# pfe-rs/lk-s-2022-estimacija-pokreta

Measured on AMD Instinct MI355X. Metric: Mpix/s flow (1024x436, bcd_times=4), higher is better.
Workload: dtype f64; 1 GPU; single 1024x436 Sintel-shape pair per step per GPU, forward only, bcd_times=4 (BASELINE.json configs[1]); cells 64x27, 150 labels/px; pairs_in_flight_per_gpu=7, mode=batch

## Files before the change

lk-s-2022-estimacija-pokreta_amd/csrc/bcd.hip:

```cpp
#include "dflow_common.h"

#define BCD_THREADS 192
#ifndef BCD_MINWAVES
#define BCD_MINWAVES 5
#endif
#define BCD_MASK_WORDS 5
#define BCD_BLK 5
#define BCD_LIST 15
#define BCD_LDS_LABELS 256
#define BCD_TB_STEPS 32
#define BCD_GROUPS 3
#define BCD_CAP_B01 40
#define BCD_CAP_B2 16
#define BCD_CAP_C01 24
#define BCD_CAP_C2 8
#define BCD_ROW_B (2 * BCD_CAP_B01 + BCD_CAP_B2)
#define BCD_ROW_C (2 * BCD_CAP_C01 + BCD_CAP_C2)
#define BCD_ROW_BC (BCD_ROW_B + BCD_ROW_C + 2)
#define BCD_POOL_DIV 32

#define BLK_MORE 0x800u
#define BLK_HAS_B 0x8000u
#define BLK_HAS_C 0x80000u
#define BLK_EMPTY_X 0xFFFFFFFFu
#define BLK_EMPTY_Y 0x000000FFu

__device__ static inline void chain_geom(int phase, int chain, int H, int W, int &ty, int &tx, int &ys, int &xs, int &len)
{
    if (phase == 0) { ty = 0; tx = 2 * chain; ys = 1; xs = 0; len = H; }
    else if (phase == 1) { ty = 2 * chain; tx = W - 1; ys = 0; xs = -1; len = W; }
    else if (phase == 2) { ty = H - 1; tx = (W / 2) * 2 - 1 - 2 * chain; ys = -1; xs = 0; len = H; }
    else { ty = (H / 2) * 2 - 1 - 2 * chain; tx = 0; ys = 0; xs = 1; len = W; }
}

struct BcdPlanes {
    uint8_t *back;
    uint2 *lab;
    uint2 *blkA;
    uint2 *blkBC;
    uint32_t *masks;
    uint32_t *cursor;
    uint32_t pool_rows;
};

__global__ void __launch_bounds__(256) bcd_lists_kernel(int H, int W, int LP, int tpsi, const uint32_t *__restrict__ proposals,
                                                        const float *__restrict__ lcosts, const int32_t *__restrict__ nprop,
                                                        BcdPlanes pl)
{
    __shared__ uint32_t s_cols[4][256];
    __shared__ __attribute__((aligned(16))) uint8_t s_list[4][64][16];
    const int lane = threadIdx.x & 63, wv = threadIdx.x >> 6;
    const int q = (int)blockIdx.x * 4 + __builtin_amdgcn_readfirstlane(wv);
    if (q >= H * W) return;
    const int y = q / W, x = q % W;
    const int py = (x & 1) ? y + 1 : y - 1, sy = (x & 1) ? y - 1 : y + 1;
    const int px = (y & 1) ? x - 1 : x + 1, sx = (y & 1) ? x + 1 : x - 1;
    const bool start0 = py < 0 || py >= H, start1 = px < 0 || px >= W;
    const bool v0 = sy >= 0 && sy < H, v1 = sx >= 0 && sx < W;
    const int p0 = v0 ? sy * W + x : q, p1 = v1 ? y * W + sx : q;
    const int pn = nprop[q], tn0 = v0 ? nprop[p0] : 0, tn1 = v1 ? nprop[p1] : 0;
    const int half = lane >> 5;
    uint32_t fq[3], f[5];
#pragma unroll
    for (int j = 0; j < 3; j++) {
        const int k = lane + 64 * j;
        fq[j] = k < pn ? flow_bias(proposals[(size_t)q * LP + k]) : 0u;
        s_cols[wv][k] = fq[j];
    }
    s_cols[wv][192 + lane] = 0u;
#pragma unroll
    for (int j = 0; j < 2; j++) {
        const int k = lane + 64 * j;
        f[j] = k < tn0 ? flow_bias(proposals[(size_t)p0 * LP + k]) : 0u;
        f[2 + j] = k < tn1 ? flow_bias(proposals[(size_t)p1 * LP + k]) : 0u;
    }
    {
        const int k = 128 + (lane & 31);
        f[4] = k < (half ? tn1 : tn0) ? flow_bias(proposals[(size_t)(half ? p1 : p0) * LP + k]) : 0u;
    }
#pragma unroll
    for (int j = 0; j < 3; j++) {
        const int k = lane + 64 * j;
        if (k < LP) pl.lab[(size_t)q * LP + k] = make_uint2(fq[j], __float_as_uint(k < pn ? lcosts[(size_t)q * LP + k] : DFLOW_FILL_COST));
    }
    if (start0 || start1) {
#pragma unroll
        for (int j = 0; j < 3; j++) {
            const int k = lane + 64 * j;
            if (k < LP) {
                if (start0) pl.blkA[((size_t)q * 2 + 0) * LP + k] = make_uint2(BLK_EMPTY_X, BLK_EMPTY_Y);
                if (start1) pl.blkA[((size_t)q * 2 + 1) * LP + k] = make_uint2(BLK_EMPTY_X, BLK_EMPTY_Y);
            }
        }
    }
    if (!v0 && !v1) return;
    const uint32_t kbias = 0x80000000u - (uint32_t)tpsi;
    const uint32_t *__restrict__ colp = proposals + (size_t)q * LP;
    uint32_t m[5][BCD_MASK_WORDS];
    const bool fifth = LP > 128 && (tn0 > 128 || tn1 > 128);
    auto build = [&](auto with5) {
#pragma unroll
        for (int j = 0; j < BCD_MASK_WORDS; j++) {
#pragma unroll
            for (int g = 0; g < 5; g++) m[g][j] = 0xFFFFFFFFu;
            if (32 * j < pn) {
                const int nv = pn - 32 * j;
                auto cols8 = [&](auto hic) {
#pragma unroll
                    for (int cc = decltype(hic)::value; cc > decltype(hic)::value - 8; cc--) {
                        const uint32_t col = flow_bias(colp[32 * j + cc]);
#pragma unroll
                        for (int g = 0; g < 4; g++) m[g][j] = __builtin_amdgcn_alignbit(m[g][j], __builtin_amdgcn_sad_u16(col, f[g], kbias), 31);
                        if (decltype(with5)::value) m[4][j] = __builtin_amdgcn_alignbit(m[4][j], __builtin_amdgcn_sad_u16(col, f[4], kbias), 31);
                    }
                };
                if (nv > 24) cols8(IntC<31>());
                if (nv > 16) cols8(IntC<23>());
                if (nv > 8) cols8(IntC<15>());
                cols8(IntC<7>());
                if (nv < 32 && (nv & 7) != 0) {
                    const uint32_t inval = ~0u << nv;
#pragma unroll
                    for (int g = 0; g < 5; g++) m[g][j] |= inval;
                }
            }
        }
    };
    if (fifth) build(IntC<1>()); else build(IntC<0>());

    auto emit = [&](auto mergedc, const uint32_t (&mg)[BCD_MASK_WORDS], const uint32_t me, const int ig, const int tl, const int tn,
                    const bool valid, const size_t pd) {
        constexpr bool MERGED = decltype(mergedc)::value != 0;
        uint32_t w[BCD_MASK_WORDS];
        int cnt = 0;
        uint32_t dead = valid && tl < tn ? 0u : ~0u;
        asm("" : "+v"(dead));
#pragma unroll
        for (int j = 0; j < BCD_MASK_WORDS; j++) { w[j] = __builtin_amdgcn_bitop3_b32(mg[j], dead, 0u, 0x03); cnt += __popc(w[j]); }
        uint8_t *row = &s_list[wv][lane][0];
        *reinterpret_cast<uint4 *>(row) = make_uint4(0xFFFFFFFFu, 0xFFFFFFFFu, 0xFFFFFFFFu, 0xFFFFFFFFu);
        const int n = min(cnt, BCD_LIST);
        const bool any = __ballot(cnt > 0) != 0ull;
        if (any) {
            uint32_t wt[BCD_MASK_WORDS];
#pragma unroll
            for (int j = 0; j < BCD_MASK_WORDS; j++) wt[j] = w[j];
            if (__ballot(cnt > BCD_LIST)) {
                int extra = cnt - BCD_LIST;
#pragma unroll
                for (int j = BCD_MASK_WORDS - 1; j >= 0; j--)
                    while (extra > 0 && wt[j]) { wt[j] &= ~(0x80000000u >> __clz(wt[j])); extra--; }
            }
            uint8_t *ap = row;
#pragma unroll
            for (int j = 0; j < BCD_MASK_WORDS; j++) {
                uint32_t ww = wt[j];
                while (ww) { *ap++ = (uint8_t)(32 * j + __ffs(ww) - 1); ww &= ww - 1; }
            }
        }
        const uint4 lst = *reinterpret_cast<const uint4 *>(row);
        const uint32_t l0 = lst.x, l1 = lst.y, l2 = lst.z, l3 = lst.w;
        uint32_t c0 = 0u, c1 = 0u;
        if (any) {
            auto slots = [&](auto lo, auto hi) {
#pragma unroll
                for (int e = decltype(lo)::value; e < decltype(hi)::value; e++) {
                    const uint32_t word = e < 4 ? l0 : (e < 8 ? l1 : (e < 12 ? l2 : l3));
                    const uint32_t k = (word >> (8 * (e & 3))) & 0xFFu;
                    const uint32_t psi = flow_l1_biased(me, s_cols[wv][k]);
                    if (e < 8) c0 |= psi << (4 * e); else c1 |= psi << (4 * (e - 8));
                }
            };
            slots(IntC<0>(), IntC<BCD_BLK>());
            if (__ballot(n > BCD_BLK)) {
                slots(IntC<BCD_BLK>(), IntC<2 * BCD_BLK>());
                if (__ballot(n > 2 * BCD_BLK)) slots(IntC<2 * BCD_BLK>(), IntC<BCD_LIST>());
            }
        }
        const unsigned long long pp = (((unsigned long long)c1 << 32) | c0) & ~(~0ull << (4 * n));
        const unsigned long long hasB = __ballot(cnt > BCD_BLK), hasC = __ballot(cnt > 2 * BCD_BLK);
        uint32_t rankB = __builtin_amdgcn_mbcnt_hi((uint32_t)(hasB >> 32), __builtin_amdgcn_mbcnt_lo((uint32_t)hasB, 0u));
        uint32_t rankC = __builtin_amdgcn_mbcnt_hi((uint32_t)(hasC >> 32), __builtin_amdgcn_mbcnt_lo((uint32_t)hasC, 0u));
        if (MERGED && half) { rankB -= (uint32_t)__popc((uint32_t)hasB); rankC -= (uint32_t)__popc((uint32_t)hasC); }
        const uint32_t capB = ig < 2 ? BCD_CAP_B01 : BCD_CAP_B2, capC = ig < 2 ? BCD_CAP_C01 : BCD_CAP_C2;
        const bool storeB = cnt > BCD_BLK && rankB < capB, storeC = cnt > 2 * BCD_BLK && storeB && rankC < capC;
        const bool more = cnt > BCD_LIST || (cnt > BCD_BLK && !storeB) || (cnt > 2 * BCD_BLK && !storeC);
        const uint32_t ax = l0;
        const uint32_t ay = (l1 & 0xFFu) | (((uint32_t)pp & 0xFFFFFu) << 8) | (more ? BLK_MORE : 0u) | (storeB ? BLK_HAS_B : 0u) |
                            (storeC ? BLK_HAS_C : 0u) | ((uint32_t)(more ? 15 : min(cnt, 15)) << 28);
        const uint32_t bx = __builtin_amdgcn_alignbit(l2, l1, 8);
        const uint32_t by = ((l2 >> 8) & 0xFFu) | (((uint32_t)(pp >> 20) & 0xFFFFFu) << 8);
        const uint32_t cx = __builtin_amdgcn_alignbit(l3, l2, 16);
        const uint32_t cy = ((l3 >> 16) & 0xFFu) | (((uint32_t)(pp >> 40) & 0xFFFFFu) << 8);
        if (valid && tl < LP) pl.blkA[pd * (size_t)LP + tl] = make_uint2(ax, ay);
        if (storeB) pl.blkBC[pd * BCD_ROW_BC + ig * BCD_CAP_B01 + rankB] = make_uint2(bx, by);
        if (storeC) pl.blkBC[pd * BCD_ROW_BC + BCD_ROW_B + ig * BCD_CAP_C01 + rankC] = make_uint2(cx, cy);
        const unsigned long long dense = __ballot(more);
        if (dense) {
            uint32_t base = 0u;
            if (lane == 0) base = atomicAdd(pl.cursor, (uint32_t)__popcll(dense));
            base = (uint32_t)__builtin_amdgcn_readfirstlane((int)base);
            uint32_t rank = __builtin_amdgcn_mbcnt_hi((uint32_t)(dense >> 32), __builtin_amdgcn_mbcnt_lo((uint32_t)dense, 0u));
            if (MERGED) {
                const uint32_t nlo = (uint32_t)__popc((uint32_t)dense);
                if ((lane & 31) == 0 && (half ? (dense >> 32) != 0ull : (uint32_t)dense != 0u))
                    reinterpret_cast<uint32_t *>(pl.blkBC + pd * BCD_ROW_BC + BCD_ROW_B + BCD_ROW_C)[ig] = base + (half ? nlo : 0u);
            } else if (lane == 0) {
                reinterpret_cast<uint32_t *>(pl.blkBC + pd * BCD_ROW_BC + BCD_ROW_B + BCD_ROW_C)[ig] = base;
            }
            const uint32_t slot = base + rank;
            if (more && slot < pl.pool_rows) {
                uint32_t *out = pl.masks + (size_t)slot * BCD_MASK_WORDS;
#pragma unroll
                for (int j = 0; j < BCD_MASK_WORDS; j++) out[j] = w[j];
            }
        }
    };
    const size_t pd0 = (size_t)p0 * 2 + 0, pd1 = (size_t)p1 * 2 + 1;
    if (v0) {
        emit(IntC<0>(), m[0], f[0], 0, lane, tn0, true, pd0);
        if (LP > 64) emit(IntC<0>(), m[1], f[1], 1, 64 + lane, tn0, true, pd0);
    }
    if (v1) {
        emit(IntC<0>(), m[2], f[2], 0, lane, tn1, true, pd1);
        if (LP > 64) emit(IntC<0>(), m[3], f[3], 1, 64 + lane, tn1, true, pd1);
    }
    if (LP > 128) emit(IntC<1>(), m[4], f[4], 2, 128 + (lane & 31), half ? tn1 : tn0, half ? v1 : v0, half ? pd1 : pd0);
}

#ifndef BCD_MAX_BATCH
#define BCD_MAX_BATCH 8
#endif
struct BcdPass {
    const int32_t *nprop;
    int32_t *bestlabels;
    BcdPlanes pl;
};
struct BcdArgs {
    int H, W, LP, tpsi, phase;
    double lamda;
    BcdPass pass[BCD_MAX_BATCH];
};

struct Cand {
    double v; int k;
};

__device__ static inline void cand_min(Cand &a, double ov, int ok)
{
    const bool take = ov < a.v || (ov == a.v && ok < a.k);
    a.v = take ? ov : a.v;
    a.k = take ? ok : a.k;
}

template <int CTRL> __device__ static inline void cand_dpp(const Cand &a, double &ov, int &ok)
{
    const int lo = __double2loint(a.v), hi = __double2hiint(a.v);
    const int olo = __builtin_amdgcn_update_dpp(lo, lo, CTRL, 0xF, 0xF, false);
    const int ohi = __builtin_amdgcn_update_dpp(hi, hi, CTRL, 0xF, 0xF, false);
    ok = __builtin_amdgcn_update_dpp(a.k, a.k, CTRL, 0xF, 0xF, false);
    ov = __hiloint2double(ohi, olo);
}

#define DPP_ROW_SHL1 0x101
#define DPP_ROW_SHL2 0x102
#define DPP_ROW_SHL4 0x104
#define DPP_ROW_SHL8 0x108

__device__ static inline void wave_min_lane0(Cand &pm)
{
    double ov; int ok;
    cand_dpp<DPP_ROW_SHL1>(pm, ov, ok); cand_min(pm, ov, ok);
    cand_dpp<DPP_ROW_SHL2>(pm, ov, ok); cand_min(pm, ov, ok);
    cand_dpp<DPP_ROW_SHL4>(pm, ov, ok); cand_min(pm, ov, ok);
    cand_dpp<DPP_ROW_SHL8>(pm, ov, ok); cand_min(pm, ov, ok);
    const int lo = __double2loint(pm.v), hi = __double2hiint(pm.v);
#pragma unroll
    for (int r = 1; r < 4; r++) {
        const double rv = __hiloint2double(__builtin_amdgcn_readlane(hi, 16 * r), __builtin_amdgcn_readlane(lo, 16 * r));
        const int rk = __builtin_amdgcn_readlane(pm.k, 16 * r);
        cand_min(pm, rv, rk);
    }
}

__device__ static inline uint32_t wave_u32_min_asm(uint32_t x)
{
    asm volatile("s_nop 1\n\t"
                 "v_min_u32_dpp %0, %0, %0 row_shl:1 row_mask:0xf bank_mask:0xf\n\t"
                 "s_nop 1\n\t"
                 "v_min_u32_dpp %0, %0, %0 row_shl:2 row_mask:0xf bank_mask:0xf\n\t"
                 "s_nop 1\n\t"
                 "v_min_u32_dpp %0, %0, %0 row_shl:4 row_mask:0xf bank_mask:0xf\n\t"
                 "s_nop 1\n\t"
                 "v_min_u32_dpp %0, %0, %0 row_shl:8 row_mask:0xf bank_mask:0xf\n\t"
                 "s_nop 0"
                 : "+v"(x));
    const uint32_t a = (uint32_t)__builtin_amdgcn_readlane((int)x, 0), b = (uint32_t)__builtin_amdgcn_readlane((int)x, 16);
    const uint32_t c = (uint32_t)__builtin_amdgcn_readlane((int)x, 32), d = (uint32_t)__builtin_amdgcn_readlane((int)x, 48);
    const uint32_t ab = a < b ? a : b, cd = c < d ? c : d;
    return ab < cd ? ab : cd;
}
__device__ static inline unsigned long long wave_key_min_asm(unsigned long long key, int *first_lane)
{
    const uint32_t hi = (uint32_t)(key >> 32), lo = (uint32_t)key;
    const uint32_t mh = wave_u32_min_asm(hi);
    const unsigned long long tie = __ballot(hi == mh);
    uint32_t ml; int fl;
    fl = __ffsll((long long)tie) - 1;
    ml = (uint32_t)__builtin_amdgcn_readlane((int)lo, fl);
    if (__builtin_expect(__popcll(tie) != 1, 0)) {
        ml = wave_u32_min_asm(hi == mh ? lo : 0xFFFFFFFFu);
        fl = __ffsll((long long)__ballot(hi == mh && lo == ml)) - 1;
    }
    *first_lane = fl;
    return ((unsigned long long)mh << 32) | ml;
}

__device__ static inline uint32_t lane_rank(unsigned long long mask)
{
    return __builtin_amdgcn_mbcnt_hi((uint32_t)(mask >> 32), __builtin_amdgcn_mbcnt_lo((uint32_t)mask, 0u));
}

#define BCD_BACK_PITCH BCD_THREADS

typedef const __attribute__((address_space(1))) char *gptr_t;
__device__ static inline gptr_t uniform_ptr(const void *p)
{
    const unsigned long long v = (unsigned long long)p;
    const uint32_t lo = __builtin_amdgcn_readfirstlane((uint32_t)v), hi = __builtin_amdgcn_readfirstlane((uint32_t)(v >> 32));
    return (gptr_t)(((unsigned long long)hi << 32) | lo);
}
__device__ static inline unsigned long long ballot64(bool b) { return __builtin_amdgcn_ballot_w64(b); }

__global__ void __launch_bounds__(BCD_THREADS, BCD_MINWAVES) bcd_chain_kernel(BcdArgs a)
{
    __shared__ double s_dp[2 * BCD_LDS_LABELS];
    __shared__ unsigned long long permv[2 * 4];
    __shared__ int permi[2 * 4 + 4];
    __shared__ __attribute__((aligned(16))) uint8_t tb[BCD_TB_STEPS * BCD_BACK_PITCH];
    extern __shared__ __attribute__((aligned(16))) uint32_t s_dyn[];
    uint32_t *bestf = s_dyn + 1;
    int *tnl;
    int *s_label = permi + 8;

    const int tid = threadIdx.x, lane = tid & 63, wave = __builtin_amdgcn_readfirstlane(tid >> 6);
    const int chain = blockIdx.x;
    const int W = a.W, LP = a.LP;
    const bool owner = tid < LP;
    const unsigned long long ownmask = ballot64(owner);
    const int tl = owner ? tid : LP - 1;
    int ty0, tx0, ys, xs, len;
    chain_geom(a.phase, chain, a.H, W, ty0, tx0, ys, xs, len);
    const int pstep = ys * W + xs;
    const int pix0 = ty0 * W + tx0;
    const int dir = ys != 0 ? 0 : 1;
    const int dirp = ys + xs;
    const uint32_t tpsi = (uint32_t)a.tpsi;
    const double tpsi_d = (double)a.tpsi;
    const double lamda = a.lamda;
    const BcdPass &ps = a.pass[blockIdx.y];
    const int32_t *g_nprop = ps.nprop;
    int32_t *g_best = ps.bestlabels;
    const uint2 *g_lab = ps.pl.lab;
    const uint32_t *g_masks = ps.pl.masks;
    const uint2 *g_bc = ps.pl.blkBC;
    const uint32_t pool_rows = ps.pl.pool_rows;
    uint8_t *back = ps.pl.back + ((size_t)chain * len) * BCD_BACK_PITCH;

    tnl = (int *)(bestf + len + 2);
    for (int i = tid; i < 2 * BCD_LDS_LABELS; i += BCD_THREADS) s_dp[i] = 1e300;
    for (int i = tid; i < len; i += BCD_THREADS) {
        int pix = pix0 + i * pstep;
        bestf[i] = g_lab[(size_t)pix * LP + g_best[pix]].x;
        tnl[i] = g_nprop[pix];
    }
    if (tid == 0) { bestf[-1] = 0u; bestf[len] = 0u; bestf[len + 1] = 0u; }
    __syncthreads();

    const uint32_t offl = (uint32_t)tl * 8u;
    const long long rowl = (long long)LP * 8, rowg = (long long)BCD_ROW_BC * 8;
    const long long strA = (long long)pstep * 2 * rowl, strL = (long long)pstep * rowl, strG = (long long)pstep * 2 * rowg;
    gptr_t pA = uniform_ptr((const char *)ps.pl.blkA + ((long long)pix0 * 2 + dir) * rowl);
    gptr_t pL = uniform_ptr((const char *)ps.pl.lab + (long long)pix0 * rowl);
    gptr_t pB = uniform_ptr((const char *)ps.pl.blkBC + ((long long)pix0 * 2 + dir) * rowg + (long long)wave * (BCD_CAP_B01 * 8));
    const uint32_t coff = (uint32_t)(BCD_ROW_B * 8 + wave * (BCD_CAP_C01 * 8) - wave * (BCD_CAP_B01 * 8));
    int nextA = 0, nextG = 0;
    auto advA = [&]() { const bool m = nextA + 1 < len; pA += m ? strA : 0; pL += m ? strL : 0; nextA++; };
    auto advG = [&]() { const bool m = nextG + 1 < len; pB += m ? strG : 0; nextG++; };
    auto ld8 = [](gptr_t base, uint32_t off) {
        const unsigned long long v = *reinterpret_cast<const __attribute__((address_space(1))) unsigned long long *>(base + off);
        return make_uint2((uint32_t)v, (uint32_t)(v >> 32));
    };
    auto fetchBC = [&](const uint2 &blkA, uint2 &B, uint2 &C) {
        const bool hb = owner && (blkA.y & BLK_HAS_B) != 0u, hc = owner && (blkA.y & BLK_HAS_C) != 0u;
        const unsigned long long mb = ballot64(hb);
        B = make_uint2(BLK_EMPTY_X, BLK_EMPTY_Y); C = make_uint2(BLK_EMPTY_X, BLK_EMPTY_Y);
        if (mb) {
            if (hb) B = ld8(pB, lane_rank(mb) * 8u);
            const unsigned long long mc = ballot64(hc);
            if (mc) { if (hc) C = ld8(pB, coff + lane_rank(mc) * 8u); }
        }
        advG();
    };
    uint2 A0, L0 = ld8(pL, offl); advA();
    uint2 A1 = ld8(pA, offl), L1 = ld8(pL, offl); advA();
    uint2 A2 = ld8(pA, offl), L2 = ld8(pL, offl); advA();
    uint2 A3 = ld8(pA, offl), L3 = ld8(pL, offl); advA();
    uint2 B1, C1, B0, C0;
    advG();
    fetchBC(A1, B1, C1);
    fetchBC(A2, B0, C0);

    {
        const uint32_t Fc = L0.x;
        const int ip = dirp, im = -dirp;
        const uint32_t s1 = (ip >= 0 && ip < len) ? min(tpsi, flow_l1_biased(Fc, bestf[ip])) : 0u;
        const uint32_t s2 = (im >= 0 && im < len) ? min(tpsi, flow_l1_biased(Fc, bestf[im])) : 0u;
        unsigned long long key = ~0ull;
        if (owner && tl < tnl[0]) {
            const double d0 = __dadd_rn((double)(s1 + s2), __dmul_rn(lamda, (double)__uint_as_float(L0.y)));
            s_dp[tl] = d0;
            key = (unsigned long long)__double_as_longlong(__dadd_rn(tpsi_d, d0));
        }
        int fl;
        const unsigned long long m = wave_key_min_asm(key, &fl);
        if (lane == 0) { permv[wave] = m; permi[wave] = wave * 64 + fl; }
    }
    A0 = ld8(pA, offl); L0 = ld8(pL, offl); advA();
    __syncthreads();

    int pn = tnl[0];
    __attribute__((address_space(1))) uint8_t *backrow = (__attribute__((address_space(1))) uint8_t *)uniform_ptr(back + BCD_BACK_PITCH);
    int tn_nx = tnl[1];
    uint32_t bfp_nx = bestf[1 + dirp], bfm_nx = bestf[1 - dirp];
    auto step = [&](auto curc, auto edgec, const int i, uint2 &inA, uint2 &inL, uint2 &inB, uint2 &inC, const uint2 &nxA) __attribute__((always_inline)) {
        constexpr int CUR = decltype(curc)::value;
        constexpr bool EDGE = decltype(edgec)::value != 0;
        const char *prev = reinterpret_cast<const char *>(s_dp + (CUR ^ 1) * BCD_LDS_LABELS);
        const int tn = tn_nx;
        const uint32_t bfp = bfp_nx, bfm = bfm_nx;
        tn_nx = tnl[min(i + 1, len - 1)];
        bfp_nx = bestf[i + 1 + dirp]; bfm_nx = bestf[i + 1 - dirp];
        const uint32_t ax = inA.x, ay = inA.y, bx = inB.x, by = inB.y, cx = inC.x, cy = inC.y;
        const uint32_t Fc = inL.x;
        const float lc = __uint_as_float(inL.y);
        const unsigned long long actmask = ballot64(tl < tn) & ownmask;
        const bool act = owner && tl < tn;
        uint32_t ad[BCD_BLK]; double dd[BCD_BLK];
#pragma unroll
        for (int j = 0; j < BCD_BLK; j++) {
            ad[j] = ((j < 4 ? ax >> (8 * j) : ay) & 0xFFu) << 3;
            dd[j] = *reinterpret_cast<const double *>(prev + ad[j]);
        }
        asm volatile("" ::: "memory");
        inA = ld8(pA, offl); inL = ld8(pL, offl); advA();
        fetchBC(nxA, inB, inC);
        Cand perm;
        double small;
        {
            const unsigned long long p0 = permv[(CUR ^ 1) * 4], p1 = permv[(CUR ^ 1) * 4 + 1], p2 = permv[(CUR ^ 1) * 4 + 2];
            const int i0 = permi[(CUR ^ 1) * 4], i1 = permi[(CUR ^ 1) * 4 + 1], i2 = permi[(CUR ^ 1) * 4 + 2];
            uint32_t lim1 = tpsi, lim2 = tpsi;
            if (EDGE) {
                const int ip = i + dirp, im = i - dirp;
                lim1 = (ip >= 0 && ip < len) ? tpsi : 0u; lim2 = (im >= 0 && im < len) ? tpsi : 0u;
            }
            const uint32_t s1 = min(flow_l1_biased(Fc, bfp), lim1);
            const uint32_t s2 = min(flow_l1_biased(Fc, bfm), lim2);
            unsigned long long pmn = p0; int pix_ = i0;
            if (p1 < pmn) { pmn = p1; pix_ = i1; }
            if (p2 < pmn) { pmn = p2; pix_ = i2; }
            perm.v = __longlong_as_double((long long)pmn); perm.k = pix_;
            small = __dadd_rn(__dadd_rn(__dmul_rn(lamda, (double)lc), (double)s1), (double)s2);
        }
        auto node = [](double &va, uint32_t &ka, const double vb, const uint32_t kb) {
            const bool t = vb < va;
            va = __builtin_fmin(va, vb); ka = t ? kb : ka;
        };
        auto block_min = [&](double (&d)[BCD_BLK], uint32_t (&k)[BCD_BLK], const uint32_t y, double &v, uint32_t &kk) {
#pragma unroll
            for (int j = 0; j < BCD_BLK; j++) d[j] = __dadd_rn(d[j], (double)((y >> (8 + 4 * j)) & 7u));
            node(d[0], k[0], d[1], k[1]); node(d[2], k[2], d[3], k[3]);
            node(d[0], k[0], d[2], k[2]); node(d[0], k[0], d[4], k[4]);
            v = d[0]; kk = k[0];
        };
        double bestv; uint32_t besta;
        block_min(dd, ad, ay, bestv, besta);
        if ((ballot64((ay >> 28) > BCD_BLK) & actmask) != 0ull) {
            uint32_t a2[BCD_BLK]; double d2[BCD_BLK];
#pragma unroll
            for (int j = 0; j < BCD_BLK; j++) { a2[j] = ((j < 4 ? bx >> (8 * j) : by) & 0xFFu) << 3; d2[j] = *reinterpret_cast<const double *>(prev + a2[j]); }
            { double vb; uint32_t kb; block_min(d2, a2, by, vb, kb); node(bestv, besta, vb, kb); }
            if (__builtin_expect((ballot64((ay >> 28) > 2 * BCD_BLK) & actmask) != 0ull, 0)) {
#pragma unroll
                for (int j = 0; j < BCD_BLK; j++) { a2[j] = ((j < 4 ? cx >> (8 * j) : cy) & 0xFFu) << 3; d2[j] = *reinterpret_cast<const double *>(prev + a2[j]); }
                { double vc; uint32_t kc; block_min(d2, a2, cy, vc, kc); node(bestv, besta, vc, kc); }
                const bool more = act && (ay & BLK_MORE) != 0u;
                const unsigned long long moremask = ballot64(more);
                if (__builtin_expect(moremask != 0ull, 0)) {
                    const int klast = (int)(((ay & BLK_HAS_C) ? cy : (ay & BLK_HAS_B) ? by : ay) & 0xFFu);
                    const size_t cpix = (size_t)(pix0 + i * pstep), ppix = (size_t)(pix0 + (i - 1) * pstep);
                    const uint2 *plab = g_lab + ppix * LP;
                    unsigned long long w0 = 0, w1 = 0, w2 = 0;
                    if (more) {
                        const uint32_t mbase = reinterpret_cast<const uint32_t *>(g_bc + (cpix * 2 + dir) * BCD_ROW_BC + BCD_ROW_B + BCD_ROW_C)[wave];
                        const uint32_t slot = mbase + lane_rank(moremask);
                        if (slot < pool_rows) {
                            const uint32_t *mrow = g_masks + (size_t)slot * BCD_MASK_WORDS;
                            w0 = (unsigned long long)mrow[0] | ((unsigned long long)mrow[1] << 32);
                            w1 = (unsigned long long)mrow[2] | ((unsigned long long)mrow[3] << 32);
                            w2 = (unsigned long long)mrow[4];
                        } else {
                            for (int k = klast + 1; k < pn; k++) {
                                const unsigned long long bit = flow_l1_biased(Fc, plab[k].x) < tpsi ? 1ull << (k & 63) : 0ull;
                                if (k < 64) w0 |= bit; else if (k < 128) w1 |= bit; else w2 |= bit;
                            }
                        }
                        const int b = klast & 63;
                        const unsigned long long keep = b == 63 ? 0ull : (~0ull << (b + 1));
                        if (klast < 64) w0 &= keep; else if (klast < 128) { w0 = 0; w1 &= keep; } else { w0 = 0; w1 = 0; w2 &= keep; }
                    }
                    int base = 0;
                    auto next_bit = [&](bool &valid) {
                        if (w0 == 0) { w0 = w1; w1 = w2; w2 = 0; base += 64; if (w0 == 0) { w0 = w1; w1 = 0; base += 64; } }
                        valid = w0 != 0;
                        int k = 0;
                        if (valid) { k = base + __ffsll((long long)w0) - 1; w0 &= w0 - 1; }
                        return k;
                    };
                    while (w0 | w1 | w2) {
                        bool v[4]; int kk[4]; double d4[4]; uint32_t ff[4];
#pragma unroll
                        for (int j = 0; j < 4; j++) kk[j] = next_bit(v[j]);
#pragma unroll
                        for (int j = 0; j < 4; j++) { d4[j] = *reinterpret_cast<const double *>(prev + 8 * kk[j]); ff[j] = plab[kk[j]].x; }
#pragma unroll
                        for (int j = 0; j < 4; j++) {
                            const double c = __dadd_rn(d4[j], (double)flow_l1_biased(Fc, ff[j]));
                            const bool t = v[j] && c < bestv;
                            bestv = t ? c : bestv; besta = t ? (uint32_t)kk[j] << 3 : besta;
                        }
                    }
                }
            }
        }
        unsigned long long key;
        {
            const bool found = bestv < 1e300;
            const double mincost = found ? bestv : perm.v;
            const int pl_ = found ? (int)(besta >> 3) : perm.k;
            const double dpc = __dadd_rn(mincost, small);
            s_dp[CUR * BCD_LDS_LABELS + tid] = dpc;
            backrow[tid] = (uint8_t)pl_;
            backrow += BCD_BACK_PITCH;
            key = act ? (unsigned long long)__double_as_longlong(__dadd_rn(tpsi_d, dpc)) : ~0ull;
        }
        {
            int fl;
            const unsigned long long m = wave_key_min_asm(key, &fl);
            if (lane == 0) { permv[CUR * 4 + wave] = m; permi[CUR * 4 + wave] = wave * 64 + fl; }
        }
        asm volatile("s_waitcnt lgkmcnt(0)" ::: "memory");
        __builtin_amdgcn_s_barrier();
        asm volatile("" ::: "memory");
        pn = tn;
    };
    int i = 1;
    for (; i + 4 < len; i += 4) {
        step(IntC<1>(), IntC<0>(), i, A1, L1, B1, C1, A3);
        step(IntC<0>(), IntC<0>(), i + 1, A2, L2, B0, C0, A0);
        step(IntC<1>(), IntC<0>(), i + 2, A3, L3, B1, C1, A1);
        step(IntC<0>(), IntC<0>(), i + 3, A0, L0, B0, C0, A2);
    }
    if (i < len) step(IntC<1>(), IntC<1>(), i, A1, L1, B1, C1, A3);
    if (i + 1 < len) step(IntC<0>(), IntC<1>(), i + 1, A2, L2, B0, C0, A0);
    if (i + 2 < len) step(IntC<1>(), IntC<1>(), i + 2, A3, L3, B1, C1, A1);
    if (i + 3 < len) step(IntC<0>(), IntC<1>(), i + 3, A0, L0, B0, C0, A2);
    const int cur = (len & 1) ? 1 : 0;

    if (tid < 64) {
        const double *dp = s_dp + (cur ^ 1) * BCD_LDS_LABELS;
        Cand m; m.v = 800000.0; m.k = 0x7fffffff;
        for (int k = lane; k < pn; k += 64) { double c = dp[k]; if (c < m.v) { m.v = c; m.k = k; } }
        wave_min_lane0(m);
        if (tid == 0) *s_label = m.k == 0x7fffffff ? 0 : m.k;
    }
    __syncthreads();
    int plb = *s_label;
    if (tid == 0) g_best[pix0 + (len - 1) * pstep] = plb;
    for (int hi = len - 1; hi >= 1; hi -= BCD_TB_STEPS) {
        const int lo = max(1, hi - BCD_TB_STEPS + 1);
        const int nbytes = (hi - lo + 1) * BCD_BACK_PITCH;
        const uint4 *src = reinterpret_cast<const uint4 *>(back + (size_t)lo * BCD_BACK_PITCH);
        for (int j = tid; j < nbytes / 16; j += BCD_THREADS) reinterpret_cast<uint4 *>(tb)[j] = src[j];
        __syncthreads();
        if (tid == 0) {
            for (int i2 = hi; i2 >= lo; i2--) {
                plb = tb[(i2 - lo) * BCD_BACK_PITCH + plb];
                g_best[pix0 + (i2 - 1) * pstep] = plb;
            }
            *s_label = plb;
        }
        __syncthreads();
        plb = *s_label;
    }
}

static void phase_dims(const dflow_params *p, int phase, int &nchains, int &len)
{
    int H = p->pich, W = p->picw;
    if (phase == 0) { nchains = (W + 1) / 2; len = H; }
    else if (phase == 1) { nchains = (H + 1) / 2; len = W; }
    else if (phase == 2) { nchains = W / 2; len = H; }
    else { nchains = H / 2; len = W; }
}

static uint32_t pool_rows_of(const dflow_params *p)
{
    const size_t rows = (size_t)p->pich * p->picw * 2 * p->label_pitch / BCD_POOL_DIV;
    return (uint32_t)(rows < 4096 ? 4096 : rows);
}

static BcdPlanes planes_of(const dflow_params *p, void *ws, size_t *bytes = nullptr)
{
    const size_t n = (size_t)p->pich * p->picw;
    size_t back = 0;
    for (int ph = 0; ph < 4; ph++) {
        int nchains, len;
        phase_dims(p, ph, nchains, len);
        const size_t b = (size_t)nchains * len * BCD_BACK_PITCH;
        if (b > back) back = b;
    }
    WsCarver c(ws);
    BcdPlanes pl;
    pl.pool_rows = pool_rows_of(p);
    pl.back = c.take<uint8_t>(back);
    pl.lab = c.take<uint2>(n * p->label_pitch);
    pl.blkA = c.take<uint2>(n * 2 * p->label_pitch);
    pl.blkBC = c.take<uint2>(n * 2 * BCD_ROW_BC);
    pl.masks = c.take<uint32_t>((size_t)pl.pool_rows * BCD_MASK_WORDS);
    pl.cursor = c.take<uint32_t>(256 / sizeof(uint32_t));
    if (bytes) *bytes = c.bytes;
    return pl;
}

size_t bcd_ws_bytes(const dflow_params *p) { size_t b; planes_of(p, nullptr, &b); return b; }

int launch_bcd_prepare(const dflow_params *p, const uint32_t *proposals, const float *lcosts, const int32_t *nprop, void *ws,
                       hipStream_t s)
{
    long long items = (long long)p->pich * p->picw;
    DFLOW_HIP(hipMemsetAsync(planes_of(p, ws).cursor, 0, 256, s));
    hipLaunchKernelGGL(bcd_lists_kernel, dim3((unsigned)((items + 3) / 4)), dim3(256), 0, s, p->pich, p->picw, p->label_pitch,
                       p->tpsi, proposals, lcosts, nprop, planes_of(p, ws));
    return dflow_check_launch("bcd_lists_kernel");
}

int launch_bcd_phase_batch(const dflow_params *p, int npass, const int32_t *const *nprop, int32_t *const *bestlabels, int phase,
                           void *const *ws, hipStream_t s)
{
    int nchains, len;
    phase_dims(p, phase, nchains, len);
    if (nchains == 0) return DFLOW_OK;
    size_t shmem = (size_t)(len + 4) * sizeof(uint32_t) + (size_t)len * sizeof(int);
    for (int b0 = 0; b0 < npass; b0 += BCD_MAX_BATCH) {
        const int nb = npass - b0 < BCD_MAX_BATCH ? npass - b0 : BCD_MAX_BATCH;
        BcdArgs a;
        a.H = p->pich; a.W = p->picw; a.LP = p->label_pitch; a.tpsi = p->tpsi; a.phase = phase; a.lamda = p->lamda;
        for (int b = 0; b < BCD_MAX_BATCH; b++) {
            const int src = b0 + (b < nb ? b : 0);
            a.pass[b].nprop = nprop[src]; a.pass[b].bestlabels = bestlabels[src]; a.pass[b].pl = planes_of(p, ws[src]);
        }
        hipLaunchKernelGGL(bcd_chain_kernel, dim3(nchains, nb), dim3(BCD_THREADS), shmem, s, a);
        int rc = dflow_check_launch("bcd_chain_kernel");
        if (rc) return rc;
    }
    return DFLOW_OK;
}

int launch_bcd_phase(const dflow_params *p, const int32_t *nprop, int32_t *bestlabels, int phase, void *ws, hipStream_t s)
{
    void *wsv = ws;
    return launch_bcd_phase_batch(p, 1, &nprop, &bestlabels, phase, &wsv, s);
}
```

Before: 41.97 Mpix/s.

## Build label neighborhood masks via rotated-coordinate counting sort and prefix-OR sets

Replaces the brute-force pairwise label comparison in bcd_lists_kernel with a range-query scheme. Proposals are mapped to two rotated coordinates (u+v, u-v), counting-sorted in per-wave LDS, and prefix-OR bitsets are built so each neighbor's L1-ball mask comes from two table lookups per axis. The old path is kept as a fallback when the coordinate spread exceeds the table range. LDS per wave grows to 4 KB and launch bounds now request 8 waves, which may limit occupancy and adds more wave-level synchronisation.

Measured after the change: 43.37 Mpix/s (median of 6 runs). 3.3% higher.

```diff
diff --git a/lk-s-2022-estimacija-pokreta_amd/csrc/bcd.hip b/lk-s-2022-estimacija-pokreta_amd/csrc/bcd.hip
--- a/lk-s-2022-estimacija-pokreta_amd/csrc/bcd.hip
+++ b/lk-s-2022-estimacija-pokreta_amd/csrc/bcd.hip
@@ -43,12 +43,96 @@
     uint32_t pool_rows;
 };
 
-__global__ void __launch_bounds__(256) bcd_lists_kernel(int H, int W, int LP, int tpsi, const uint32_t *__restrict__ proposals,
+#ifndef BCD_RANGE_BYTES
+#define BCD_RANGE_BYTES 768
+#endif
+#define BCD_RANGE_R (BCD_RANGE_BYTES - 1)
+#ifndef BCD_RANGE_PITCH
+#define BCD_RANGE_PITCH 5
+#endif
+#define BCD_RANGE_ENTRIES (DFLOW_MAX_LABELS + 1)
+#ifndef BCD_LISTS_WAVE_LDS
+#define BCD_LISTS_WAVE_LDS 4096
+#endif
+static_assert(BCD_RANGE_BYTES % 256 == 0 && BCD_RANGE_BYTES >= 256 && BCD_RANGE_BYTES <= 1024, "rank table: 1..4 dwords per lane");
+static_assert(BCD_RANGE_BYTES + BCD_RANGE_ENTRIES * BCD_RANGE_PITCH * 4 <= BCD_LISTS_WAVE_LDS && BCD_LISTS_WAVE_LDS >= 1024, "a wave's LDS");
+static_assert(BCD_RANGE_PITCH >= BCD_MASK_WORDS && BCD_RANGE_PITCH <= 8, "prefix-set entry pitch");
+
+__device__ static inline void wave_lds_sync()
+{
+    __builtin_amdgcn_fence(__ATOMIC_RELEASE, "wavefront");
+    __builtin_amdgcn_wave_barrier();
+    __builtin_amdgcn_fence(__ATOMIC_ACQUIRE, "wavefront");
+}
+template <int CTRL, int ROWS = 0xF> __device__ static inline uint32_t dpp_or0(uint32_t v)
+{
+    return (uint32_t)__builtin_amdgcn_update_dpp(0, (int)v, CTRL, ROWS, 0xF, false);
+}
+__device__ static inline uint32_t wave_scan_add(uint32_t x)
+{
+    x += dpp_or0<0x111>(x); x += dpp_or0<0x112>(x); x += dpp_or0<0x114>(x); x += dpp_or0<0x118>(x);
+    x += dpp_or0<0x142, 0xA>(x); x += dpp_or0<0x143, 0xC>(x);
+    return x;
+}
+template <int CTRL, int ROWS = 0xF> __device__ static inline void sets_or_step(uint32_t (&x)[BCD_MASK_WORDS])
+{
+#pragma unroll
+    for (int w = 0; w < BCD_MASK_WORDS; w++) x[w] |= dpp_or0<CTRL, ROWS>(x[w]);
+}
+__device__ static inline void wave_scan_or(uint32_t (&x)[BCD_MASK_WORDS])
+{
+    sets_or_step<0x111>(x); sets_or_step<0x112>(x); sets_or_step<0x114>(x); sets_or_step<0x118>(x);
+    sets_or_step<0x142, 0xA>(x); sets_or_step<0x143, 0xC>(x);
+}
+template <int CTRL, int ROWS = 0xF> __device__ static inline int dpp_min(int v)
+{
+    return min(v, __builtin_amdgcn_update_dpp(v, v, CTRL, ROWS, 0xF, false));
+}
+__device__ static inline int wave_min(int x)
+{
+    x = dpp_min<0x111>(x); x = dpp_min<0x112>(x); x = dpp_min<0x114>(x); x = dpp_min<0x118>(x);
+    x = dpp_min<0x142, 0xA>(x); x = dpp_min<0x143, 0xC>(x);
+    return __builtin_amdgcn_readlane(x, 63);
+}
+__device__ static inline void sets_load(const uint32_t *e, uint32_t (&w)[BCD_MASK_WORDS])
+{
+    if constexpr (BCD_RANGE_PITCH % 4 == 0) {
+        const uint4 a = *reinterpret_cast<const uint4 *>(e);
+        w[0] = a.x; w[1] = a.y; w[2] = a.z; w[3] = a.w;
+    } else if constexpr (BCD_RANGE_PITCH % 2 == 0) {
+        const uint2 a = *reinterpret_cast<const uint2 *>(e), b = *reinterpret_cast<const uint2 *>(e + 2);
+        w[0] = a.x; w[1] = a.y; w[2] = b.x; w[3] = b.y;
+    } else {
+        w[0] = e[0]; w[1] = e[1]; w[2] = e[2]; w[3] = e[3];
+    }
+    w[4] = e[4];
+}
+__device__ static inline void sets_store(uint32_t *e, const uint32_t (&w)[BCD_MASK_WORDS])
+{
+    if constexpr (BCD_RANGE_PITCH % 4 == 0) {
+        *reinterpret_cast<uint4 *>(e) = make_uint4(w[0], w[1], w[2], w[3]);
+    } else if constexpr (BCD_RANGE_PITCH % 2 == 0) {
+        *reinterpret_cast<uint2 *>(e) = make_uint2(w[0], w[1]); *reinterpret_cast<uint2 *>(e + 2) = make_uint2(w[2], w[3]);
+    } else {
+        e[0] = w[0]; e[1] = w[1]; e[2] = w[2]; e[3] = w[3];
+    }
+    e[4] = w[4];
+}
+template <int AX> __device__ static inline int range_coord(uint32_t f)
+{
+    const int lo = (int)(f & 0xFFFFu), hi = (int)(f >> 16);
+    return AX ? lo - hi + 65535 : lo + hi;
+}
+
+#ifndef BCD_LISTS_WAVES
+#define BCD_LISTS_WAVES 8
+#endif
+__global__ void __launch_bounds__(256, BCD_LISTS_WAVES) bcd_lists_kernel(int H, int W, int LP, int tpsi, const uint32_t *__restrict__ proposals,
                                                         const float *__restrict__ lcosts, const int32_t *__restrict__ nprop,
                                                         BcdPlanes pl)
 {
     __shared__ uint32_t s_cols[4][256];
-    __shared__ __attribute__((aligned(16))) uint8_t s_list[4][64][16];
+    __shared__ __attribute__((aligned(16))) uint8_t s_wave[4][BCD_LISTS_WAVE_LDS];
     const int lane = threadIdx.x & 63, wv = threadIdx.x >> 6;
     const int q = (int)blockIdx.x * 4 + __builtin_amdgcn_readfirstlane(wv);
     if (q >= H * W) return;
@@ -126,7 +210,115 @@
             }
         }
     };
-    if (fifth) build(IntC<1>()); else build(IntC<0>());
+    const int pt = min(pn, DFLOW_MAX_LABELS);
+    int cq[2][3], org[2];
+    bool wide = false;
+#pragma unroll
+    for (int j = 0; j < 3; j++) { cq[0][j] = range_coord<0>(fq[j]); cq[1][j] = range_coord<1>(fq[j]); }
+#pragma unroll
+    for (int ax = 0; ax < 2; ax++) {
+        int mn = 1 << 18;
+#pragma unroll
+        for (int j = 0; j < 3; j++) if (lane + 64 * j < pt) mn = min(mn, cq[ax][j]);
+        org[ax] = wave_min(mn);
+#pragma unroll
+        for (int j = 0; j < 3; j++) { cq[ax][j] -= org[ax]; wide |= lane + 64 * j < pt && cq[ax][j] >= BCD_RANGE_R; }
+    }
+    if (__ballot(wide)) {
+        if (fifth) build(IntC<1>()); else build(IntC<0>());
+    } else {
+        constexpr int NW = BCD_RANGE_BYTES / 256;
+        uint32_t *const cw = reinterpret_cast<uint32_t *>(&s_wave[wv][0]);
+        const uint8_t *const cb = &s_wave[wv][0];
+        uint32_t *const sets = reinterpret_cast<uint32_t *>(&s_wave[wv][BCD_RANGE_BYTES]);
+        auto axis = [&](auto axc) {
+            constexpr int AX = decltype(axc)::value;
+#pragma unroll
+            for (int i = 0; i < NW; i++) cw[lane * NW + i] = 0u;
+            wave_lds_sync();
+            uint32_t ord[3];
+#pragma unroll
+            for (int j = 0; j < 3; j++) {
+                ord[j] = 0u;
+                if (lane + 64 * j < pt) {
+                    const uint32_t rel = (uint32_t)cq[AX][j], sh = 8u * (rel & 3u);
+                    ord[j] = (atomicAdd(&cw[rel >> 2], 1u << sh) >> sh) & 0xFFu;
+                }
+            }
+            wave_lds_sync();
+            uint32_t t[NW], before[NW], tot = 0u;
+#pragma unroll
+            for (int i = 0; i < NW; i++) {
+                t[i] = cw[lane * NW + i];
+                t[i] += t[i] << 8; t[i] += t[i] << 16;
+                before[i] = tot; tot += t[i] >> 24;
+            }
+            const uint32_t lower = wave_scan_add(tot) - tot;
+#pragma unroll
+            for (int i = 0; i < NW; i++) {
+                const uint32_t base = lower + before[i];
+                cw[lane * NW + i] = (t[i] << 8) + __builtin_amdgcn_perm(base, base, 0x00000000u);
+            }
+            if (lane == 0) {
+                const uint32_t none[BCD_MASK_WORDS] = {0u, 0u, 0u, 0u, 0u};
+                sets_store(sets, none);
+            }
+            wave_lds_sync();
+#pragma unroll
+            for (int j = 0; j < 3; j++) {
+                if (lane + 64 * j < pt) {
+                    const uint32_t r = (uint32_t)cb[cq[AX][j]] + ord[j], bit = 1u << (lane & 31);
+                    uint32_t one[BCD_MASK_WORDS] = {0u, 0u, 0u, 0u, 0u};
+                    one[2 * j] = half ? 0u : bit;
+                    if (j < 2) one[2 * j + 1] = half ? bit : 0u;
+                    sets_store(sets + (r + 1u) * BCD_RANGE_PITCH, one);
+                }
+            }
+            wave_lds_sync();
+            uint32_t a[3][BCD_MASK_WORDS];
+#pragma unroll
+            for (int i = 0; i < 3; i++) {
+#pragma unroll
+                for (int w = 0; w < BCD_MASK_WORDS; w++) a[i][w] = 0u;
+                if (3 * lane + i <= pt) sets_load(sets + (3 * lane + i) * BCD_RANGE_PITCH, a[i]);
+            }
+#pragma unroll
+            for (int w = 0; w < BCD_MASK_WORDS; w++) { a[1][w] |= a[0][w]; a[2][w] |= a[1][w]; }
+            wave_scan_or(a[2]);
+#pragma unroll
+            for (int w = 0; w < BCD_MASK_WORDS; w++) {
+                const uint32_t lower_lanes = dpp_or0<0x138>(a[2][w]);
+                a[0][w] |= lower_lanes; a[1][w] |= lower_lanes;
+            }
+#pragma unroll
+            for (int i = 0; i < 3; i++)
+                if (3 * lane + i <= pt) sets_store(sets + (3 * lane + i) * BCD_RANGE_PITCH, a[i]);
+            wave_lds_sync();
+#pragma unroll
+            for (int g = 0; g < 5; g++) {
+                if (g < 4 || fifth) {
+                    const int c = range_coord<AX>(f[g]) - org[AX];
+                    const int hi = min(max(c + tpsi, 0), BCD_RANGE_R), lo = min(max(c - tpsi + 1, 0), BCD_RANGE_R);
+                    uint32_t in[BCD_MASK_WORDS], out[BCD_MASK_WORDS];
+                    sets_load(sets + (uint32_t)cb[hi] * BCD_RANGE_PITCH, in);
+                    sets_load(sets + (uint32_t)cb[lo] * BCD_RANGE_PITCH, out);
+#pragma unroll
+                    for (int w = 0; w < BCD_MASK_WORDS; w++) {
+                        if (AX == 0) m[g][w] = in[w] & ~out[w];
+                        else m[g][w] = ~(m[g][w] & in[w] & ~out[w]);
+                        asm("" : "+v"(m[g][w]));
+                    }
+                } else {
+#pragma unroll
+                    for (int w = 0; w < BCD_MASK_WORDS; w++) m[g][w] = 0xFFFFFFFFu;
+                }
+                if (g & 1) __builtin_amdgcn_sched_barrier(0);
+            }
+            wave_lds_sync();
+        };
+        axis(IntC<0>());
+        axis(IntC<1>());
+    }
 
     auto emit = [&](auto mergedc, const uint32_t (&mg)[BCD_MASK_WORDS], const uint32_t me, const int ig, const int tl, const int tn,
                     const bool valid, const size_t pd) {
@@ -137,7 +329,7 @@
         asm("" : "+v"(dead));
 #pragma unroll
         for (int j = 0; j < BCD_MASK_WORDS; j++) { w[j] = __builtin_amdgcn_bitop3_b32(mg[j], dead, 0u, 0x03); cnt += __popc(w[j]); }
-        uint8_t *row = &s_list[wv][lane][0];
+        uint8_t *row = &s_wave[wv][16 * lane];
         *reinterpret_cast<uint4 *>(row) = make_uint4(0xFFFFFFFFu, 0xFFFFFFFFu, 0xFFFFFFFFu, 0xFFFFFFFFu);
         const int n = min(cnt, BCD_LIST);
         const bool any = __ballot(cnt > 0) != 0ull;
```
